# CIS565-Fall-2014/Project3-Pathtracer

Measured on NVIDIA B200. Metric: path segments per second, reference sample scene 800x800, 5000 spp, 8 bounces, higher is better.
Workload: dtype f32

## Files before the change

project3-pathtracer_b200/csrc/pt_api.cu:

```cuda
#include "../../include/pt_b200.h"
#include "pt_kernels.cuh"

#include <nvtx3/nvToolsExt.h>

#include <cmath>
#include <cstdarg>
#include <cstdio>
#include <cstring>
#include <string>
#include <algorithm>
#include <atomic>
#include <thread>
#include <functional>
#include <vector>

using namespace ptd;

struct NvtxRange {
  explicit NvtxRange(const char* name) { nvtxRangePushA(name); }
  ~NvtxRange() { nvtxRangePop(); }
};

static thread_local std::string g_err;
extern "C" void pt_set_error_(const char* fmt, ...) {
// ... 28 lines not shown
  int sm_count = 0;
  cudaStream_t own_stream = nullptr, stream = nullptr;
  cudaEvent_t ev0 = nullptr, ev1 = nullptr;
  bool timed = false;
  int n_geoms = 0, n_mats = 0;
  float4* d_rows = nullptr;
  int2* d_meta = nullptr;
  float4* d_normals = nullptr;
  float4* d_mats = nullptr;
  float4* d_lights = nullptr;
  float* d_light_k = nullptr;
  int n_lights = 0;
  bool nee = false;
  float4* d_filt = nullptr;
  int2* d_filt_ids = nullptr;
  FiltSoA filt{};
  int filt_cap = 0;
  float4* d_bvh_nodes = nullptr;
  float4* d_bvh_leaves = nullptr;
  int2* d_bvh_meta = nullptr;
  BvhSoA bvh{};
  float filter_scale = 1.0f;
  std::vector<pt_static_geom> h_geoms;
  GeomSoA g{};
  RaygenConsts cam{};
  uint32_t W = 0, H = 0, npix = 0;
  uint64_t wf_capacity = 0;
  uint32_t band_pixels = 0;
#ifndef PT_WF_SLOTS
#define PT_WF_SLOTS 2
// ... 531 lines not shown

template <bool F, bool L>
static int setup_variant(pt_context* c, int slot) {
  int per_sm = 0, per_sm_nee = 0;
  constexpr bool N = NeeOf<F, L>::value;
  if (c->mode) {
    CU(cudaFuncSetAttribute(k_bounce_bvh<L>, cudaFuncAttributeMaxDynamicSharedMemorySize, (int)kBvhSmemBytes));
    CU(cudaOccupancyMaxActiveBlocksPerMultiprocessor(&per_sm, k_bounce_bvh<L>, kBvhThreads, kBvhSmemBytes));
    CU(cudaFuncSetAttribute(k_bounce_bvh<L, N>, cudaFuncAttributeMaxDynamicSharedMemorySize, (int)kBvhSmemBytes));
    CU(cudaOccupancyMaxActiveBlocksPerMultiprocessor(&per_sm_nee, k_bounce_bvh<L, N>, kBvhThreads, kBvhSmemBytes));
  } else {
    CU(cudaFuncSetAttribute(k_bounce<F, L>, cudaFuncAttributeMaxDynamicSharedMemorySize, (int)c->smem_bytes));
    CU(cudaOccupancyMaxActiveBlocksPerMultiprocessor(&per_sm, k_bounce<F, L>, kBounceThreads, c->smem_bytes));
    CU(cudaFuncSetAttribute(k_bounce<F, L, N>, cudaFuncAttributeMaxDynamicSharedMemorySize, (int)c->smem_bytes));
    CU(cudaOccupancyMaxActiveBlocksPerMultiprocessor(&per_sm_nee, k_bounce<F, L, N>, kBounceThreads, c->smem_bytes));
  }
  if (per_sm < 1 || per_sm_nee < 1) { pt_set_error_("k_bounce does not fit on an SM"); return PT_ERR_CUDA; }
  c->grid_blocks[slot] = per_sm * c->sm_count;
  c->grid_blocks_nee[slot] = per_sm_nee * c->sm_count;
  return PT_OK;
}

template <bool L>
static int setup_variant_q(pt_context* c, int slot) {
  int per_sm = 0, per_sm_nee = 0;
  constexpr bool N = true;
  CU(cudaFuncSetAttribute(k_bounce_q<L>, cudaFuncAttributeMaxDynamicSharedMemorySize, (int)c->q_smem_total));
  CU(cudaFuncSetAttribute(k_bounce_q<L>, cudaFuncAttributePreferredSharedMemoryCarveout, cudaSharedmemCarveoutMaxShared));
  CU(cudaOccupancyMaxActiveBlocksPerMultiprocessor(&per_sm, k_bounce_q<L>, kQThreads, c->q_smem_total));
  CU(cudaFuncSetAttribute(k_bounce_q<L, N>, cudaFuncAttributeMaxDynamicSharedMemorySize, (int)c->q_smem_total));
// ... 86 lines not shown
  if (c->d_bvh_leaves) CU(cudaFree(c->d_bvh_leaves));
  if (c->d_bvh_meta) CU(cudaFree(c->d_bvh_meta));
  c->d_bvh_nodes = nullptr; c->d_bvh_leaves = nullptr; c->d_bvh_meta = nullptr;
  c->bvh = BvhSoA{};
  if (!F.leaf_meta.empty()) {
    CU(cudaMalloc(&c->d_bvh_nodes, F.nodes.size() * sizeof(float4)));
    CU(cudaMalloc(&c->d_bvh_leaves, F.leaves.size() * sizeof(float4)));
    CU(cudaMalloc(&c->d_bvh_meta, F.leaf_meta.size() * sizeof(int2)));
    CU(cudaMemcpy(c->d_bvh_nodes, F.nodes.data(), F.nodes.size() * sizeof(float4), cudaMemcpyHostToDevice));
    CU(cudaMemcpy(c->d_bvh_leaves, F.leaves.data(), F.leaves.size() * sizeof(float4), cudaMemcpyHostToDevice));
    CU(cudaMemcpy(c->d_bvh_meta, F.leaf_meta.data(), F.leaf_meta.size() * sizeof(int2), cudaMemcpyHostToDevice));
    c->bvh.nodes = c->d_bvh_nodes; c->bvh.leaves = c->d_bvh_leaves; c->bvh.leaf_meta = c->d_bvh_meta;
    c->bvh.n_leaves = (int)F.leaf_meta.size(); c->bvh.ew_c_max = F.ew_c_max; c->bvh.ew_w_max = F.ew_w_max;
    c->bvh.root = F.root;
  }
  return PT_OK;
}

static int upload_scene(pt_context* c, const pt_static_geom* geoms, int n_geoms, const pt_material* mats, int n_mats,
                        const pt_camera_data* cam, const pt_lens* lens, bool first) {
  if (!geoms || n_geoms <= 0 || !mats || n_mats <= 0 || !cam) {
    pt_set_error_("geoms, materials and camera are required and must be non-empty");
    return PT_ERR_INVALID;
  }
  const int Wi = (int)cam->resolution[0], Hi = (int)cam->resolution[1];
  if (Wi <= 0 || Hi <= 0 || (uint64_t)Wi * (uint64_t)Hi > (1ull << 31)) {
    pt_set_error_("bad resolution %d x %d", Wi, Hi);
    return PT_ERR_INVALID;
  }
  if (!first && ((uint32_t)Wi != c->W || (uint32_t)Hi != c->H)) {
// ... 71 lines not shown
    c->geom_smem = filt_smem_bytes(cap);
    c->mode = mode;
    c->smem_bytes = mode == 0 ? c->geom_smem : kBvhSmemBytes;
    int rc;
    if ((rc = setup_variant<true, false>(c, 0))) return rc;
    if ((rc = setup_variant<true, true>(c, 1))) return rc;
    if ((rc = setup_variant<false, false>(c, 2))) return rc;
    if ((rc = setup_variant<false, true>(c, 3))) return rc;
    if (mode == 0) {
      c->q_smem_total = c->geom_smem + q_smem_bytes();
      if ((rc = setup_variant_q<false>(c, 0))) return rc;
      if ((rc = setup_variant_q<true>(c, 1))) return rc;
    }
    CU(cudaFuncSetAttribute(k_intersect_list, cudaFuncAttributeMaxDynamicSharedMemorySize, (int)c->geom_smem));
  }
  return PT_OK;
}

static size_t state_bytes(uint64_t cap) { return (((size_t)cap * (7 * sizeof(float4))) + 255) & ~(size_t)255; }
static int alloc_wavefront(pt_context* c, uint64_t max_paths) {
  uint64_t spp = max_paths / c->npix;
  if (spp < 1) spp = 1;
  const uint64_t cap = spp * c->npix;
  if (cap > 0xFFFFFF00ull) { pt_set_error_("wavefront of %llu paths exceeds 2^32", (unsigned long long)cap); return PT_ERR_INVALID; }
  if (cap == c->wf_capacity) return PT_OK;
  int n_slots = pt_context::kSlots;
  if (const char* env = getenv("PT_B200_SLOTS")) n_slots = atoi(env) >= 2 ? pt_context::kSlots : 1;
  if (n_slots > 1 && !c->wf_stream[0]) {
    CU(cudaEventCreateWithFlags(&c->ev_fork, cudaEventDisableTiming));
    for (int i = 0; i < pt_context::kSlots; i++) {
      CU(cudaStreamCreateWithFlags(&c->wf_stream[i], cudaStreamNonBlocking));
// ... 21 lines not shown
  return PT_OK;
}

extern "C" int pt_context_destroy(pt_context* c) {
  if (!c) return PT_OK;
  cudaSetDevice(c->device);
  cudaStream_t streams[] = {c->stream, c->ahead_stream, c->copy_stream, c->wf_stream[0], c->wf_stream[1], c->own_stream};
  for (cudaStream_t st : streams)
    if (st) cudaStreamSynchronize(st);
  const bool dbg = getenv("PT_B200_DEBUG_DESTROY") != nullptr;
  auto chk = [&](cudaError_t e, const char* what) {
    if (e != cudaSuccess && dbg) fprintf(stderr, "pt_context_destroy: %s -> %s\n", what, cudaGetErrorString(e));
  };
#define PT_FREE(p) chk(cudaFree(p), #p)
  PT_FREE(c->d_rows); PT_FREE(c->d_meta); PT_FREE(c->d_normals); PT_FREE(c->d_mats); PT_FREE(c->d_lights); PT_FREE(c->d_state);
  PT_FREE(c->d_filt); PT_FREE(c->d_filt_ids); PT_FREE(c->d_bvh_nodes); PT_FREE(c->d_bvh_leaves); PT_FREE(c->d_bvh_meta);
  PT_FREE(c->d_ctrl); PT_FREE(c->d_live); PT_FREE(c->d_accum); PT_FREE(c->d_rgb); PT_FREE(c->d_rgba8);
  PT_FREE(c->d_scratch); PT_FREE(c->d_light_k); PT_FREE(c->d_shadow);
  PT_FREE(c->d_slab); PT_FREE(c->d_means); PT_FREE(c->d_base[0]); PT_FREE(c->d_base[1]);
#undef PT_FREE
  for (int i = 0; i < pt_context::kSlots; i++) {
    if (c->wf_stream[i]) chk(cudaStreamDestroy(c->wf_stream[i]), "wf_stream");
    if (c->ev_join[i]) chk(cudaEventDestroy(c->ev_join[i]), "ev_join");
  }
  if (c->ev_fork) chk(cudaEventDestroy(c->ev_fork), "ev_fork");
  if (c->ahead_stream) chk(cudaStreamDestroy(c->ahead_stream), "ahead_stream");
  if (c->copy_stream) chk(cudaStreamDestroy(c->copy_stream), "copy_stream");
  if (c->ev_res) chk(cudaEventDestroy(c->ev_res), "ev_res");
  if (c->ev_copy) chk(cudaEventDestroy(c->ev_copy), "ev_copy");
  for (int i = 0; i < 2; i++) {
    if (c->ev_ready[i]) chk(cudaEventDestroy(c->ev_ready[i]), "ev_ready");
// ... 119 lines not shown
    if (nee) k_bounce_q<L, N><<<gq, kQThreads, c->q_smem_total, st>>>(P);
    else k_bounce_q<L><<<gq, kQThreads, c->q_smem_total, st>>>(P);
  } else if (c->mode) {
    if (F) {
      const uint32_t blocks = (n_upper + 255u) / 256u, most = (uint32_t)c->sm_count * 8u;
      k_raygen_wf<<<blocks < most ? (blocks ? blocks : 1u) : most, 256, 0, st>>>(P);
      c->launches++;
    }
    const uint32_t ctas = (n_upper + kPoolMin * (kBvhThreads / 32) - 1) / (kPoolMin * (kBvhThreads / 32));
    if (ctas < grid) grid = ctas ? ctas : 1;
    if (nee) k_bounce_bvh<L, N><<<grid, kBvhThreads, kBvhSmemBytes, st>>>(P);
    else k_bounce_bvh<L><<<grid, kBvhThreads, kBvhSmemBytes, st>>>(P);
  } else {
    const uint32_t ctas = (n_upper + kBounceThreads - 1) / kBounceThreads;
    if (ctas < grid) grid = ctas ? ctas : 1;
    if (nee) k_bounce<F, L, N><<<grid, kBounceThreads, c->smem_bytes, st>>>(P);
    else k_bounce<F, L><<<grid, kBounceThreads, c->smem_bytes, st>>>(P);
  }
  c->launches++;
  return cudaGetLastError();
}

static int ensure_shadow(pt_context* c) {
  if (!(c->d_shadow && c->shadow_cap == c->wf_capacity && c->shadow_slots == c->n_slots)) {
    if (c->d_shadow) CU(cudaFree(c->d_shadow));
    c->d_shadow = nullptr; c->shadow_cap = 0;
    if (cudaMalloc(&c->d_shadow, (size_t)c->n_slots * 4 * c->wf_capacity * sizeof(float4)) != cudaSuccess) {
      const cudaError_t e = cudaGetLastError();
      c->d_shadow = nullptr;
      pt_set_error_("cudaMalloc of the shadow-ray queues (%llu paths) failed: %s", (unsigned long long)c->wf_capacity, cudaGetErrorString(e));
      return PT_ERR_CUDA;
    }
// ... 65 lines not shown
    const int sl = (int)(wf % (uint64_t)slots_used);
    cudaStream_t st = forked ? c->wf_stream[sl] : stream0;
    float4* S = reinterpret_cast<float4*>(reinterpret_cast<char*>(c->d_state) + (size_t)sl * state_bytes(cap));
    WfCtrl* ctrl = c->d_ctrl + sl;
    const uint32_t ns = (n_samples - s0 < spp_wf) ? (n_samples - s0) : spp_wf;
    const uint32_t n_first = ns * band;
    CU(cudaMemsetAsync(ctrl, 0, sizeof(WfCtrl), st));
    for (int depth = 0; depth < max_depth; depth++) {
      BounceParams P;
      const int in = depth & 1, outb = in ^ 1;
      P.in_o = S + (3 * in + 0) * cap; P.in_d = S + (3 * in + 1) * cap; P.in_t = S + (3 * in + 2) * cap;
      P.out_o = S + (3 * outb + 0) * cap; P.out_d = S + (3 * outb + 1) * cap; P.out_t = S + (3 * outb + 2) * cap;
      P.accum = accum; P.acc_s0 = acc_s0; P.acc_stride = acc_stride;
      P.g = c->g; P.n_geoms = c->n_geoms;
      P.normals = c->d_normals;
      P.filt = c->filt; P.filt_cap = c->filt_cap;
      P.bvh = c->bvh;
      P.bvh_res = S + 6 * cap;
      float4* const SQ = nee_on ? c->d_shadow + (size_t)sl * 4 * cap : nullptr;
      P.sq_o = SQ; P.sq_d = SQ ? SQ + cap : nullptr; P.sq_t = SQ ? SQ + 2 * cap : nullptr; P.sq_x = SQ ? SQ + 3 * cap : nullptr;
      P.mats = c->d_mats;
      P.lights = c->d_lights; P.n_lights = c->n_lights; P.light_k = c->d_light_k;
      P.cam = c->cam;
      P.ctrl = ctrl;
      P.depth = (uint32_t)depth;
      P.keys = philox_keys(seed);
      P.first_sample = first_sample + s0;
      P.n_first = n_first;
      P.pix0 = pix0; P.band = band;
      P.div_band = make_fastdiv(band);
      P.q_offset = (uint32_t)c->geom_smem;
// ... 297 lines not shown
  CU(cudaMemcpyAsync(&fb, dfb, sizeof(fb), cudaMemcpyDeviceToHost, c->stream));
  CU(cudaStreamSynchronize(c->stream));
  if (fallbacks) *fallbacks = fb;
  return PT_OK;
}
extern "C" int pt_intersect(pt_context* c, int n, const float* origin, const float* direction, int32_t* geom_id,
                            float* t, float* point, float* normal) {
  return pt_intersect_ex(c, PT_HIT_FILTERED, n, origin, direction, geom_id, t, point, normal, nullptr);
}

extern "C" int pt_set_filter_scale(pt_context* c, float scale) {
  CTX(c);
  if (!(scale >= 0.0f) || !(scale <= 1e6f)) { pt_set_error_("filter scale %g outside [0, 1e6]", (double)scale); return PT_ERR_INVALID; }
  CU(cudaStreamSynchronize(c->stream));
  c->filter_scale = scale;
  return upload_filter(c);
}

extern "C" int pt_filter_stats(pt_context* c, uint64_t* fallbacks) {
  CTX(c);
  if (!fallbacks) { pt_set_error_("fallbacks is NULL"); return PT_ERR_INVALID; }
  unsigned long long h = 0;
  CU(cudaMemcpyAsync(&h, c->d_live + kMaxDepth, sizeof(h), cudaMemcpyDeviceToHost, c->stream));
  CU(cudaStreamSynchronize(c->stream));
  *fallbacks = h;
  return PT_OK;
}

extern "C" int pt_filter_retries(pt_context* c, uint64_t* retries) {
  CTX(c);
  if (!retries) { pt_set_error_("retries is NULL"); return PT_ERR_INVALID; }
// ... 283 lines not shown
```

project3-pathtracer_b200/csrc/pt_filter.cuh:

```cuda
#pragma once
#include "pt_device.cuh"

namespace ptd {

__device__ __forceinline__ float mufu_rcp(float x) { float y; asm("rcp.approx.ftz.f32 %0, %1;" : "=f"(y) : "f"(x)); return y; }
__device__ __forceinline__ float mufu_sqrt(float x) { float y; asm("sqrt.approx.ftz.f32 %0, %1;" : "=f"(y) : "f"(x)); return y; }

constexpr int kFiltRows = 10;
constexpr int kFiltClasses = 4;
struct FiltSoA {
  const float4* rows;
  const int2* ids;
  int end[kFiltClasses];
  float r_scene;
};
__host__ __device__ inline size_t filt_smem_bytes(int cap) { return (size_t)cap * kFiltRows * sizeof(float4); }
__device__ __forceinline__ void stage_filt(const FiltSoA& g, int first, int count, float4* smem) {
  for (int i = threadIdx.x; i < count * kFiltRows; i += blockDim.x) smem[i] = g.rows[(size_t)first * kFiltRows + i];
}

typedef float2 f2;
__device__ __forceinline__ f2 bc2(float x) { return make_float2(x, x); }
__device__ __forceinline__ f2 lo2(float4 v) { return make_float2(v.x, v.y); }
__device__ __forceinline__ f2 hi2(float4 v) { return make_float2(v.z, v.w); }
// ... 39 lines not shown
  const bool first = lo < b.lo1, second = !first && lo < b.lo2;
  b.lo3 = first || second ? b.lo2 : fminf(b.lo3, lo);
  b.lo2 = first ? b.lo1 : (second ? lo : b.lo2);
  b.k2 = first ? b.k1 : (second ? k : b.k2);
  b.lo1 = first ? lo : b.lo1;
  b.k1 = first ? k : b.k1;
}
__device__ __forceinline__ void scan_take(ScanBest& b, float lo, int k) {
  lo = fmaxf(lo, 0.0f);
  const bool better = lo < b.lo1;
  b.lo2 = fminf(b.lo2, better ? b.lo1 : lo);
  b.k1 = better ? k : b.k1;
  b.lo1 = fminf(b.lo1, lo);
}

#define PT_FILT_TRANSFORM(V, R)                                                                          \
  const float4 Q0 = (V)[0], Q1 = (V)[1], Q2 = (V)[2], Q3 = (V)[3], Q4 = (V)[4], Q5 = (V)[5];             \
  const f2 rox = fma2(lo2(Q0), bc2((R).o.x), fma2(hi2(Q0), bc2((R).o.y), fma2(lo2(Q1), bc2((R).o.z), hi2(Q1)))); \
  const f2 roy = fma2(lo2(Q2), bc2((R).o.x), fma2(hi2(Q2), bc2((R).o.y), fma2(lo2(Q3), bc2((R).o.z), hi2(Q3)))); \
  const f2 roz = fma2(lo2(Q4), bc2((R).o.x), fma2(hi2(Q4), bc2((R).o.y), fma2(lo2(Q5), bc2((R).o.z), hi2(Q5)))); \
  const f2 rwx = fma2(lo2(Q0), bc2((R).d.x), fma2(hi2(Q0), bc2((R).d.y), mul2(lo2(Q1), bc2((R).d.z))));          \
  const f2 rwy = fma2(lo2(Q2), bc2((R).d.x), fma2(hi2(Q2), bc2((R).d.y), mul2(lo2(Q3), bc2((R).d.z))));          \
  const f2 rwz = fma2(lo2(Q4), bc2((R).d.x), fma2(hi2(Q4), bc2((R).d.y), mul2(lo2(Q5), bc2((R).d.z))));

#define PT_SPHERE_HALF(H)                                                                             \
  const float sd_##H = mufu_sqrt(disc.H), ia_##H = mufu_rcp(a.H);                                     \
  const bool miss_##H = (disc.H < 0.0f) || ((sd_##H - b.H) * ia_##H < 0.0f);  \
  const float lo_##H = __fmaf_rn((-b.H - sd_##H) * ia_##H, r.dl, -ew.H);
#define PT_BOX_HALF(H)                                                                                \
  const float tnear_##H = fmaxf(fmaxf(nx.H, ny.H), nz.H), tfar_##H = fminf(fminf(fx.H, fy.H), fz.H);  \
  const bool miss_##H = (tnear_##H > tfar_##H) || (tfar_##H < 0.0f);  \
  const float lo_##H = __fmaf_rn(tnear_##H, r.dl, -ew.H);
template <typename Sink>
__device__ __forceinline__ void filter_scan_to(const float4* v, int first, int last, const int end[kFiltClasses],
                                               const ScanRay& r, Sink& sink) {
  int i = first;
  const f2 w2 = bc2(r.w);
  for (const int e = min(last, end[0]); i < e; i++, v += kFiltRows) {
    const float4 C0 = v[0], C1 = v[1], C2 = v[2], C3 = v[3];
    const f2 ocx = __fadd2_rn(bc2(r.o.x), neg2(lo2(C0))), ocy = __fadd2_rn(bc2(r.o.y), neg2(hi2(C0))),
             ocz = __fadd2_rn(bc2(r.o.z), neg2(lo2(C1)));
    const f2 b = fma2(ocx, bc2(r.d.x), fma2(ocy, bc2(r.d.y), mul2(ocz, bc2(r.d.z))));
    const f2 oc2 = fma2(ocx, ocx, fma2(ocy, ocy, mul2(ocz, ocz)));
    const f2 R2 = fma2(hi2(C2), oc2, fma2(lo2(C2), w2, hi2(C1)));
    const f2 nc = __fadd2_rn(R2, neg2(oc2));
    const f2 disc = fma2(bc2(r.a), nc, mul2(b, b));
    if (disc.x < 0.0f && disc.y < 0.0f) continue;
    const f2 ew = fma2(hi2(C3), w2, lo2(C3));
    const f2 a = bc2(r.a);
    PT_SPHERE_HALF(x)
    PT_SPHERE_HALF(y)
    sink(lo_x, miss_x, lo_y, miss_y, i);
  }
  for (const int e = min(last, end[1]); i < e; i++, v += kFiltRows) {
    PT_FILT_TRANSFORM(v, r)
    const float4 K0 = v[6], K1 = v[7];
    const f2 a = fma2(rwx, rwx, fma2(rwy, rwy, mul2(rwz, rwz)));
    const f2 b = fma2(rox, rwx, fma2(roy, rwy, mul2(roz, rwz)));
    const f2 ro2 = fma2(rox, rox, fma2(roy, roy, mul2(roz, roz)));
    const f2 R2 = fma2(lo2(K1), ro2, fma2(hi2(K0), w2, lo2(K0)));
    const f2 nc = __fadd2_rn(R2, neg2(ro2));
    const f2 disc = fma2(a, nc, mul2(b, b));
    if (disc.x < 0.0f && disc.y < 0.0f) continue;
    const f2 ew = fma2(lo2(v[8]), w2, hi2(K1));
    PT_SPHERE_HALF(x)
    PT_SPHERE_HALF(y)
    sink(lo_x, miss_x, lo_y, miss_y, i);
  }
  for (const int e = min(last, end[2]); i < e; i++, v += kFiltRows) {
    const float4 C0 = v[0], C1 = v[1], C2 = v[2], C3 = v[3], C4 = v[4];
    const f2 cx = fma2(lo2(C0), bc2(r.id.x), bc2(-r.od.x)), cy = fma2(hi2(C0), bc2(r.id.y), bc2(-r.od.y)),
             cz = fma2(lo2(C1), bc2(r.id.z), bc2(-r.od.z));
    const f2 hx = fma2(lo2(C3), w2, hi2(C1)), hy = fma2(hi2(C3), w2, lo2(C2)), hz = fma2(lo2(C4), w2, hi2(C2));
    const f2 aix = bc2(fabsf(r.id.x)), aiy = bc2(fabsf(r.id.y)), aiz = bc2(fabsf(r.id.z));
    const f2 nx = fma2(hx, neg2(aix), cx), ny = fma2(hy, neg2(aiy), cy), nz = fma2(hz, neg2(aiz), cz);
    const f2 fx = fma2(hx, aix, cx), fy = fma2(hy, aiy, cy), fz = fma2(hz, aiz, cz);
    const f2 ew = fma2(lo2(v[5]), w2, hi2(C4));
    PT_BOX_HALF(x)
    PT_BOX_HALF(y)
    sink(lo_x, miss_x, lo_y, miss_y, i);
  }
  for (const int e = min(last, end[3]); i < e; i++, v += kFiltRows) {
    PT_FILT_TRANSFORM(v, r)
    const float4 K0 = v[6], K1 = v[7], K2 = v[8], K3 = v[9];
    const f2 hx = fma2(hi2(K1), w2, lo2(K0)), hy = fma2(lo2(K2), w2, hi2(K0)), hz = fma2(hi2(K2), w2, lo2(K1));
    const f2 ix = make_float2(mufu_rcp(rwx.x), mufu_rcp(rwx.y)), iy = make_float2(mufu_rcp(rwy.x), mufu_rcp(rwy.y)),
             iz = make_float2(mufu_rcp(rwz.x), mufu_rcp(rwz.y));
    const f2 cx = mul2(neg2(rox), ix), cy = mul2(neg2(roy), iy), cz = mul2(neg2(roz), iz);
    const f2 nx = fma2(hx, neg2(abs2(ix)), cx), ny = fma2(hy, neg2(abs2(iy)), cy), nz = fma2(hz, neg2(abs2(iz)), cz);
    const f2 fx = fma2(hx, abs2(ix), cx), fy = fma2(hy, abs2(iy), cy), fz = fma2(hz, abs2(iz), cz);
    const f2 ew = fma2(hi2(K3), w2, lo2(K3));
    PT_BOX_HALF(x)
    PT_BOX_HALF(y)
    sink(lo_x, miss_x, lo_y, miss_y, i);
  }
}
#undef PT_SPHERE_HALF
#undef PT_BOX_HALF
#undef PT_FILT_TRANSFORM
#ifndef PT_FILT_KEYED
#define PT_FILT_KEYED 1
#endif
struct TakeBest {
  ScanBest& b;
  __device__ __forceinline__ void operator()(float lo_a, bool miss_a, float lo_b, bool miss_b, int pair) {
    scan_take(b, miss_a ? INFINITY : lo_a, 2 * pair);
    scan_take(b, miss_b ? INFINITY : lo_b, 2 * pair + 1);
  }
};
constexpr int kKeyBits = 7;
constexpr uint32_t kKeyMask = (1u << kKeyBits) - 1u;
struct TakeBestKeyed {
  float k1 = INFINITY, k2 = INFINITY;
  static __device__ __forceinline__ float key(float lo, bool miss, uint32_t k) {
    const float v = __uint_as_float((__float_as_uint(fmaxf(lo, 0.0f)) & ~kKeyMask) | k);
    return miss ? INFINITY : v;
  }
  __device__ __forceinline__ void operator()(float lo_a, bool miss_a, float lo_b, bool miss_b, int pair) {
    const float ka = key(lo_a, miss_a, 2u * pair), kb = key(lo_b, miss_b, 2u * pair + 1u);
    const float mn = fminf(ka, kb), mx = fmaxf(ka, kb);
    k2 = fminf(fminf(k2, fmaxf(k1, mn)), mx);
    k1 = fminf(k1, mn);
  }
  __device__ __forceinline__ void finish(ScanBest& b) const {
    b.k1 = k1 < INFINITY ? (int)(__float_as_uint(k1) & kKeyMask) : -1;
    b.lo1 = __uint_as_float(__float_as_uint(k1) & ~kKeyMask);
    b.lo2 = __uint_as_float(__float_as_uint(k2) & ~kKeyMask);
  }
};
__device__ __forceinline__ void filter_scan(const float4* v, int first, int last, const int end[kFiltClasses],
                                            const ScanRay& r, ScanBest& best) {
#if PT_FILT_KEYED
  TakeBestKeyed sink;
  filter_scan_to(v, first, last, end, r, sink);
  sink.finish(best);
#else
  TakeBest sink{best};
  filter_scan_to(v, first, last, end, r, sink);
#endif
}

template <typename M>
__device__ __forceinline__ bool exact_hit(int type, float4 i0, float4 i1, float4 i2, float4 f0, float4 f1, float4 f2,
                                          f3 o, f3 d, float& dist, f3& P, int& ncode, M& m) {
  const f3 ro = mulMV(i0, i1, i2, o.x, o.y, o.z, 1.0f);
  const f3 rd = normalize(mulMV(i0, i1, i2, d.x, d.y, d.z, 0.0f), m);
  float t;
  if (type == 0) {
    const float vDot = dot(ro, rd);
    const float radicand = (float)((double)(vDot * vDot) - ((double)dot(ro, ro) - 0.25));
    if (radicand < 0) return false;
    const float sq = m.sqrt(radicand);
    const float first_term = -vDot;
// ... 71 lines not shown
```

project3-pathtracer_b200/csrc/pt_kernels.cuh:

```cuda
#pragma once
#include "pt_device.cuh"
#include "pt_filter.cuh"
#include "pt_bvh.cuh"
#include "pt_sampling.cuh"

namespace ptd {

constexpr int kMaxDepth = 64;
constexpr int kTile = 256;
#ifndef PT_BOUNCE_THREADS
#define PT_BOUNCE_THREADS 256
#endif
constexpr int kBounceThreads = PT_BOUNCE_THREADS;
#ifndef PT_MIN_BLOCKS
#define PT_MIN_BLOCKS 4
#endif

struct WfCtrl {
  uint32_t count[kMaxDepth + 1];
  uint32_t tile_ctr[kMaxDepth + 1];
  uint32_t fallbacks;
  uint32_t retries;
  unsigned long long shadow;
  uint32_t shadow_ctr[kMaxDepth + 1];
// ... 37 lines not shown
    if (pmask) break;
    look -= 32;
  }
  if (lane == 0) st_store(status + tile, st_pack(epoch, kStPrefix, exclusive + aggregate));
  return exclusive;
}

struct BounceParams {
  const float4 *in_o, *in_d, *in_t;
  float4 *out_o, *out_d, *out_t;
  float4* accum;
  GeomSoA g;
  const float4* normals;
  int n_geoms;
  FiltSoA filt;
  int filt_cap;
  BvhSoA bvh;
  float4* bvh_res;
  const float4* mats;
  const float4* lights;
  const float* light_k;
  int n_lights;
  RaygenConsts cam;
  WfCtrl* ctrl;
  uint32_t depth;
  PhiloxKeys keys;
  uint32_t first_sample, n_first;
  uint32_t pix0, band;
  FastDiv div_band;
  float4 *sq_o, *sq_d, *sq_t, *sq_x;
  uint32_t q_offset;
// ... 207 lines not shown
      if (NEE && PT_NEE_QUEUE) slot = __shfl_sync(0xffffffffu, W->pend_raw, 0) + rank;
    } else {
      slot = __shfl_sync(0xffffffffu, base_raw, 0) + rank;
      if (alive) {
        PT_CHECK(slot < P.cap);
        __stcs(io.out_o + slot, make_float4(o.x, o.y, o.z, __uint_as_float(pixel)));
        __stcs(io.out_d + slot, make_float4(d.x, d.y, d.z, __uint_as_float(sample)));
        __stcs(io.out_t + slot, make_float4(thr.x, thr.y, thr.z, sampled ? cos_s : 0.0f));
      }
    }
    if (NEE && (PT_NEE_QUEUE ? ballot != 0u : __any_sync(0xffffffffu, sampled)))
      direct_light<TABLE, LINEAR>(P, io, fs, lane, sampled, alive, slot, ns, o, thr, pixel, sample);
  }
}

template <bool FIRST, bool LAST, bool NEE>
__device__ __forceinline__ void bounce_fused(const BounceParams& P, const DepthIO& io, const float4* fs, uint32_t lane) {
  const uint32_t n_in = FIRST ? P.n_first : P.ctrl->count[io.depth];
  if (FIRST && blockIdx.x == 0 && threadIdx.x == 0) P.ctrl->count[0] = n_in;
  const uint32_t n_units = (n_in + kUnit - 1) / kUnit;
  uint32_t* const ticket = &P.ctrl->tile_ctr[io.depth];

  uint32_t next_raw = 0;
  if (lane == 0) next_raw = atom_add_u32(ticket, 1u);

  for (;;) {
    const uint32_t unit0 = __shfl_sync(0xffffffffu, next_raw, 0) * kTicketUnits;
    if (unit0 >= n_units) break;
    if (lane == 0) next_raw = atom_add_u32(ticket, 1u);
#pragma unroll 1
    for (uint32_t unit = unit0; unit < min(unit0 + kTicketUnits, n_units); unit++) {
// ... 12 lines not shown
      } else {
        const float4 a = __ldcs(io.in_o + idx), b = __ldcs(io.in_d + idx), c = __ldcs(io.in_t + idx);
        o = mk(a.x, a.y, a.z); pixel = __float_as_uint(a.w);
        d = mk(b.x, b.y, b.z); sample = __float_as_uint(b.w);
        thr = mk(c.x, c.y, c.z);
        if (NEE) cos_b = c.w;
      }
    }

    Hit h;
    h.t = INFINITY; h.id = -1; h.p = mk(0, 0, 0); h.ncode = 0;
    if (valid) {
      ScanBest best;
      scan_init(best);
      const ScanRay ray = make_scan_ray(o, d, P.filt.r_scene, P.filt.end[2] > P.filt.end[1]);
      filter_scan(fs, 0, P.filt.end[3], P.filt.end, ray, best);
      if (resolve_scan(best, P.filt, P.g, P.n_geoms, o, d, h)) atomicAdd(&P.ctrl->fallbacks, 1u);
    }

    shade_and_compact<LAST, true, NEE>(P, io, fs, lane, valid && h.id >= 0, h, o, d, thr, pixel, sample, cos_b);
    }
  }
}

template <bool FIRST, bool LAST, bool NEE = false>
__global__ void __launch_bounds__(kBounceThreads, PT_MIN_BLOCKS) k_bounce(const __grid_constant__ BounceParams P) {
  extern __shared__ __align__(16) unsigned char smem_raw[];
  stage_filt(P.filt, 0, P.filt.end[3], reinterpret_cast<float4*>(smem_raw));
  __syncthreads();
  bounce_fused<FIRST, LAST, NEE>(P, depth_io(P), reinterpret_cast<const float4*>(smem_raw), threadIdx.x & 31u);
}

constexpr int kQCap = 96;
#ifndef PT_Q_PREFETCH
#define PT_Q_PREFETCH 1
#endif
#ifndef PT_Q_PREFETCH_EARLY
#define PT_Q_PREFETCH_EARLY 1
#endif
#ifndef PT_Q_DEFER_OUT
#define PT_Q_DEFER_OUT 1
#endif
struct QWarp {
  float4 o[kQCap];
  float4 d[kQCap];
// ... 487 lines not shown
    __syncwarp();
  }
}

constexpr float kQSurvivalMax = 0.93f;
__global__ void k_accum_counts(const WfCtrl* ctrl, unsigned long long* live_total, int max_depth, volatile int* policy) {
  int d = threadIdx.x;
  if (d < max_depth) atomicAdd(live_total + d, (unsigned long long)ctrl->count[d]);
  if (d == 0) atomicAdd(live_total + kMaxDepth, (unsigned long long)ctrl->fallbacks);
  if (d == 1) atomicAdd(live_total + kMaxDepth + 1, ctrl->shadow);
  if (d == 2) atomicAdd(live_total + kMaxDepth + 2, (unsigned long long)ctrl->retries);
  if (policy && d >= 1 && d < max_depth && ctrl->count[d - 1] >= 4096u)
    policy[d] = (float)ctrl->count[d] < kQSurvivalMax * (float)ctrl->count[d - 1] ? 1 : 2;
}

__global__ void k_normal_table(GeomSoA g, int n_geoms, const float4* mats, float4* tab) {
  const int i = blockIdx.x * blockDim.x + threadIdx.x;
  if (i >= n_geoms) return;
  const float4 f0 = g.fwd0[i], f1 = g.fwd1[i], f2 = g.fwd2[i];
  Hit h;
  h.t = 0.0f; h.id = i; h.p = mk(0, 0, 0);
  for (int face = 0; face < 6; face++) {
    h.ncode = (face % 3) | (face >= 3 ? 4 : 0);
    const f3 n = hit_normal(f0, f1, f2, h);
    tab[(size_t)i * kNormalRows + face] = make_float4(n.x, n.y, n.z, 0.0f);
    f3 p1, p2;
    float4* fr = tab + (size_t)i * kNormalRows + kFrameRow0 + 4 * face;
    hemisphere_frame(n, p1, p2);
    fr[0] = make_float4(p1.x, p1.y, p1.z, 0.0f); fr[1] = make_float4(p2.x, p2.y, p2.z, 0.0f);
    hemisphere_frame(neg(n), p1, p2);
// ... 350 lines not shown
```

Before: 29000.

## Precompute eye-origin filter rows for primary rays in pinhole scenes

When the camera is a pinhole (aperture zero) and no BVH is used, the code precomputes per-pair filter rows specialised to the fixed eye origin. An EYE-templated first-bounce kernel then reads these origin-dependent terms (transformed origin, |oc|^2 terms, half extents, ew) instead of recomputing them per ray. This cuts arithmetic in the primary-ray filter scan only, at the cost of extra kernel instantiations, an extra device buffer, and recomputing the rows whenever the scene or filter scale changes. A standalone microbenchmark file is also added.

```diff
diff --git a/profiles/microbench/const_rows.cu b/profiles/microbench/const_rows.cu
--- /dev/null
+++ b/profiles/microbench/const_rows.cu
@@ -0,0 +1,32 @@
+#include <cuda_runtime.h>
+struct Rows { float4 r[19 * 10]; int n; };
+__device__ __forceinline__ float2 lo2(float4 v) { return make_float2(v.x, v.y); }
+__device__ __forceinline__ float2 hi2(float4 v) { return make_float2(v.z, v.w); }
+__global__ void k_fixed(const __grid_constant__ Rows R, const float4* in, float2* out) {
+  const float4 a = in[threadIdx.x + blockIdx.x * blockDim.x];
+  const float2 x = make_float2(a.x, a.y), y = make_float2(a.z, a.w);
+  float2 t = __ffma2_rn(x, lo2(R.r[3]), y);
+  t = __ffma2_rn(t, y, hi2(R.r[3]));
+  t = __ffma2_rn(t, make_float2(R.r[4].x, R.r[4].x), x);
+  t = __fadd2_rn(t, lo2(R.r[4]));
+  out[threadIdx.x] = __fmul2_rn(t, hi2(R.r[4]));
+}
+__global__ void k_loop(const __grid_constant__ Rows R, const float4* in, float* out) {
+  const float4 a = in[threadIdx.x + blockIdx.x * blockDim.x];
+  const float2 o = make_float2(a.x, a.x), d = make_float2(a.y, a.y);
+  float2 acc = make_float2(0.f, 0.f);
+#pragma unroll 1
+  for (int i = 0; i < R.n; i++) {
+    const float4 C0 = R.r[i * 10], C1 = R.r[i * 10 + 1];
+    float2 t = __ffma2_rn(lo2(C0), o, hi2(C0));
+    t = __ffma2_rn(lo2(C1), t, hi2(C1));
+    if (t.x < 0.f && t.y < 0.f) continue;
+    acc = __ffma2_rn(t, d, acc);
+  }
+  out[threadIdx.x] = acc.x + acc.y;
+}
+__global__ void k_block(const __grid_constant__ Rows R, const float4* in, float2* out) {
+  const float4 a = in[threadIdx.x + blockIdx.x * blockDim.x];
+  const float4 C = R.r[blockIdx.x];
+  out[threadIdx.x] = __ffma2_rn(make_float2(a.x, a.y), lo2(C), hi2(C));
+}
diff --git a/project3-pathtracer_b200/csrc/pt_api.cu b/project3-pathtracer_b200/csrc/pt_api.cu
--- a/project3-pathtracer_b200/csrc/pt_api.cu
+++ b/project3-pathtracer_b200/csrc/pt_api.cu
@@ -66,6 +66,8 @@
   bool nee = false;
   float4* d_filt = nullptr;
   int2* d_filt_ids = nullptr;
+  float4* d_filt_eye = nullptr;
+  bool eye_rows = false;
   FiltSoA filt{};
   int filt_cap = 0;
   float4* d_bvh_nodes = nullptr;
@@ -627,6 +629,13 @@
     CU(cudaOccupancyMaxActiveBlocksPerMultiprocessor(&per_sm, k_bounce<F, L>, kBounceThreads, c->smem_bytes));
     CU(cudaFuncSetAttribute(k_bounce<F, L, N>, cudaFuncAttributeMaxDynamicSharedMemorySize, (int)c->smem_bytes));
     CU(cudaOccupancyMaxActiveBlocksPerMultiprocessor(&per_sm_nee, k_bounce<F, L, N>, kBounceThreads, c->smem_bytes));
+    int per_sm_eye = 0, per_sm_nee_eye = 0;
+    CU(cudaFuncSetAttribute(k_bounce<F, L, false, F>, cudaFuncAttributeMaxDynamicSharedMemorySize, (int)c->smem_bytes));
+    CU(cudaOccupancyMaxActiveBlocksPerMultiprocessor(&per_sm_eye, k_bounce<F, L, false, F>, kBounceThreads, c->smem_bytes));
+    CU(cudaFuncSetAttribute(k_bounce<F, L, N, F>, cudaFuncAttributeMaxDynamicSharedMemorySize, (int)c->smem_bytes));
+    CU(cudaOccupancyMaxActiveBlocksPerMultiprocessor(&per_sm_nee_eye, k_bounce<F, L, N, F>, kBounceThreads, c->smem_bytes));
+    if (per_sm_eye < per_sm) per_sm = per_sm_eye;
+    if (per_sm_nee_eye < per_sm_nee) per_sm_nee = per_sm_nee_eye;
   }
   if (per_sm < 1 || per_sm_nee < 1) { pt_set_error_("k_bounce does not fit on an SM"); return PT_ERR_CUDA; }
   c->grid_blocks[slot] = per_sm * c->sm_count;
@@ -743,6 +752,20 @@
     c->bvh.n_leaves = (int)F.leaf_meta.size(); c->bvh.ew_c_max = F.ew_c_max; c->bvh.ew_w_max = F.ew_w_max;
     c->bvh.root = F.root;
   }
+  return PT_OK;
+}
+
+static int upload_eye_rows(pt_context* c) {
+  c->eye_rows = false;
+  const int n_pairs = c->filt.end[3];
+  if (c->bvh.n_leaves > 0 || !(c->cam.aperture == 0.0f) || n_pairs < 1) return PT_OK;
+  if (c->d_filt_eye) CU(cudaFree(c->d_filt_eye));
+  c->d_filt_eye = nullptr;
+  CU(cudaMalloc(&c->d_filt_eye, (size_t)n_pairs * kFiltRows * sizeof(float4)));
+  k_eye_rows<<<(n_pairs + 127) / 128, 128, 0, c->stream>>>(c->filt, c->cam.eye, c->d_filt_eye);
+  CU(cudaGetLastError());
+  CU(cudaStreamSynchronize(c->stream));
+  c->eye_rows = true;
   return PT_OK;
 }
 
@@ -844,7 +867,7 @@
     }
     CU(cudaFuncSetAttribute(k_intersect_list, cudaFuncAttributeMaxDynamicSharedMemorySize, (int)c->geom_smem));
   }
-  return PT_OK;
+  return upload_eye_rows(c);
 }
 
 static size_t state_bytes(uint64_t cap) { return (((size_t)cap * (7 * sizeof(float4))) + 255) & ~(size_t)255; }
@@ -896,7 +919,7 @@
   };
 #define PT_FREE(p) chk(cudaFree(p), #p)
   PT_FREE(c->d_rows); PT_FREE(c->d_meta); PT_FREE(c->d_normals); PT_FREE(c->d_mats); PT_FREE(c->d_lights); PT_FREE(c->d_state);
-  PT_FREE(c->d_filt); PT_FREE(c->d_filt_ids); PT_FREE(c->d_bvh_nodes); PT_FREE(c->d_bvh_leaves); PT_FREE(c->d_bvh_meta);
+  PT_FREE(c->d_filt); PT_FREE(c->d_filt_ids); PT_FREE(c->d_filt_eye); PT_FREE(c->d_bvh_nodes); PT_FREE(c->d_bvh_leaves); PT_FREE(c->d_bvh_meta);
   PT_FREE(c->d_ctrl); PT_FREE(c->d_live); PT_FREE(c->d_accum); PT_FREE(c->d_rgb); PT_FREE(c->d_rgba8);
   PT_FREE(c->d_scratch); PT_FREE(c->d_light_k); PT_FREE(c->d_shadow);
   PT_FREE(c->d_slab); PT_FREE(c->d_means); PT_FREE(c->d_base[0]); PT_FREE(c->d_base[1]);
@@ -1046,8 +1069,16 @@
   } else {
     const uint32_t ctas = (n_upper + kBounceThreads - 1) / kBounceThreads;
     if (ctas < grid) grid = ctas ? ctas : 1;
-    if (nee) k_bounce<F, L, N><<<grid, kBounceThreads, c->smem_bytes, st>>>(P);
-    else k_bounce<F, L><<<grid, kBounceThreads, c->smem_bytes, st>>>(P);
+    if (F && c->eye_rows && (PT_NEE_QUEUE || !nee)) {
+      BounceParams Pe = P;
+      Pe.filt.rows = c->d_filt_eye;
+      if (nee) k_bounce<F, L, N, F><<<grid, kBounceThreads, c->smem_bytes, st>>>(Pe);
+      else k_bounce<F, L, false, F><<<grid, kBounceThreads, c->smem_bytes, st>>>(Pe);
+    } else if (nee) {
+      k_bounce<F, L, N><<<grid, kBounceThreads, c->smem_bytes, st>>>(P);
+    } else {
+      k_bounce<F, L><<<grid, kBounceThreads, c->smem_bytes, st>>>(P);
+    }
   }
   c->launches++;
   return cudaGetLastError();
@@ -1143,7 +1174,7 @@
       P.accum = accum; P.acc_s0 = acc_s0; P.acc_stride = acc_stride;
       P.g = c->g; P.n_geoms = c->n_geoms;
       P.normals = c->d_normals;
-      P.filt = c->filt; P.filt_cap = c->filt_cap;
+      P.filt = c->filt;
       P.bvh = c->bvh;
       P.bvh_res = S + 6 * cap;
       float4* const SQ = nee_on ? c->d_shadow + (size_t)sl * 4 * cap : nullptr;
@@ -1471,7 +1502,8 @@
   if (!(scale >= 0.0f) || !(scale <= 1e6f)) { pt_set_error_("filter scale %g outside [0, 1e6]", (double)scale); return PT_ERR_INVALID; }
   CU(cudaStreamSynchronize(c->stream));
   c->filter_scale = scale;
-  return upload_filter(c);
+  if (int rc = upload_filter(c)) return rc;
+  return upload_eye_rows(c);
 }
 
 extern "C" int pt_filter_stats(pt_context* c, uint64_t* fallbacks) {
diff --git a/project3-pathtracer_b200/csrc/pt_filter.cuh b/project3-pathtracer_b200/csrc/pt_filter.cuh
--- a/project3-pathtracer_b200/csrc/pt_filter.cuh
+++ b/project3-pathtracer_b200/csrc/pt_filter.cuh
@@ -77,14 +77,77 @@
   b.lo1 = fminf(b.lo1, lo);
 }
 
-#define PT_FILT_TRANSFORM(V, R)                                                                          \
-  const float4 Q0 = (V)[0], Q1 = (V)[1], Q2 = (V)[2], Q3 = (V)[3], Q4 = (V)[4], Q5 = (V)[5];             \
-  const f2 rox = fma2(lo2(Q0), bc2((R).o.x), fma2(hi2(Q0), bc2((R).o.y), fma2(lo2(Q1), bc2((R).o.z), hi2(Q1)))); \
-  const f2 roy = fma2(lo2(Q2), bc2((R).o.x), fma2(hi2(Q2), bc2((R).o.y), fma2(lo2(Q3), bc2((R).o.z), hi2(Q3)))); \
-  const f2 roz = fma2(lo2(Q4), bc2((R).o.x), fma2(hi2(Q4), bc2((R).o.y), fma2(lo2(Q5), bc2((R).o.z), hi2(Q5)))); \
-  const f2 rwx = fma2(lo2(Q0), bc2((R).d.x), fma2(hi2(Q0), bc2((R).d.y), mul2(lo2(Q1), bc2((R).d.z))));          \
-  const f2 rwy = fma2(lo2(Q2), bc2((R).d.x), fma2(hi2(Q2), bc2((R).d.y), mul2(lo2(Q3), bc2((R).d.z))));          \
-  const f2 rwz = fma2(lo2(Q4), bc2((R).d.x), fma2(hi2(Q4), bc2((R).d.y), mul2(lo2(Q5), bc2((R).d.z))));
+__device__ __forceinline__ void filt_ro(const float4* v, f3 o, f2& rox, f2& roy, f2& roz) {
+  const float4 Q0 = v[0], Q1 = v[1], Q2 = v[2], Q3 = v[3], Q4 = v[4], Q5 = v[5];
+  rox = fma2(lo2(Q0), bc2(o.x), fma2(hi2(Q0), bc2(o.y), fma2(lo2(Q1), bc2(o.z), hi2(Q1))));
+  roy = fma2(lo2(Q2), bc2(o.x), fma2(hi2(Q2), bc2(o.y), fma2(lo2(Q3), bc2(o.z), hi2(Q3))));
+  roz = fma2(lo2(Q4), bc2(o.x), fma2(hi2(Q4), bc2(o.y), fma2(lo2(Q5), bc2(o.z), hi2(Q5))));
+}
+__device__ __forceinline__ void filt_rw(const float4* v, f3 d, f2& rwx, f2& rwy, f2& rwz) {
+  const float4 Q0 = v[0], Q1 = v[1], Q2 = v[2], Q3 = v[3], Q4 = v[4], Q5 = v[5];
+  rwx = fma2(lo2(Q0), bc2(d.x), fma2(hi2(Q0), bc2(d.y), mul2(lo2(Q1), bc2(d.z))));
+  rwy = fma2(lo2(Q2), bc2(d.x), fma2(hi2(Q2), bc2(d.y), mul2(lo2(Q3), bc2(d.z))));
+  rwz = fma2(lo2(Q4), bc2(d.x), fma2(hi2(Q4), bc2(d.y), mul2(lo2(Q5), bc2(d.z))));
+}
+__device__ __forceinline__ void filt_origin0(const float4* v, f3 o, f2 w2, f2& ocx, f2& ocy, f2& ocz, f2& nc) {
+  const float4 C0 = v[0], C1 = v[1], C2 = v[2];
+  ocx = __fadd2_rn(bc2(o.x), neg2(lo2(C0))); ocy = __fadd2_rn(bc2(o.y), neg2(hi2(C0)));
+  ocz = __fadd2_rn(bc2(o.z), neg2(lo2(C1)));
+  const f2 oc2 = fma2(ocx, ocx, fma2(ocy, ocy, mul2(ocz, ocz)));
+  const f2 R2 = fma2(hi2(C2), oc2, fma2(lo2(C2), w2, hi2(C1)));
+  nc = __fadd2_rn(R2, neg2(oc2));
+}
+__device__ __forceinline__ f2 filt_nc1(const float4* v, f2 w2, f2 rox, f2 roy, f2 roz) {
+  const float4 K0 = v[6], K1 = v[7];
+  const f2 ro2 = fma2(rox, rox, fma2(roy, roy, mul2(roz, roz)));
+  const f2 R2 = fma2(lo2(K1), ro2, fma2(hi2(K0), w2, lo2(K0)));
+  return __fadd2_rn(R2, neg2(ro2));
+}
+__device__ __forceinline__ void filt_half2(const float4* v, f2 w2, f2& hx, f2& hy, f2& hz) {
+  const float4 C1 = v[1], C2 = v[2], C3 = v[3], C4 = v[4];
+  hx = fma2(lo2(C3), w2, hi2(C1)); hy = fma2(hi2(C3), w2, lo2(C2)); hz = fma2(lo2(C4), w2, hi2(C2));
+}
+__device__ __forceinline__ void filt_half3(const float4* v, f2 w2, f2& hx, f2& hy, f2& hz) {
+  const float4 K0 = v[6], K1 = v[7], K2 = v[8];
+  hx = fma2(hi2(K1), w2, lo2(K0)); hy = fma2(lo2(K2), w2, hi2(K0)); hz = fma2(hi2(K2), w2, lo2(K1));
+}
+template <int K>
+__device__ __forceinline__ f2 filt_ew(const float4* v, f2 w2) {
+  if (K == 0) return fma2(hi2(v[3]), w2, lo2(v[3]));
+  if (K == 1) return fma2(lo2(v[8]), w2, hi2(v[7]));
+  if (K == 2) return fma2(lo2(v[5]), w2, hi2(v[4]));
+  return fma2(hi2(v[9]), w2, lo2(v[9]));
+}
+
+__device__ __forceinline__ void eye_rows_of_pair(const FiltSoA& f, int i, f3 eye, float4* e) {
+  const float4* const v = f.rows + (size_t)i * kFiltRows;
+  for (int k = 0; k < kFiltRows; k++) e[k] = v[k];
+  const ScanRay r = make_scan_ray(eye, mk(0, 0, 1), f.r_scene, false);
+  const f2 w2 = bc2(r.w);
+  const f2 z = bc2(0.0f);
+  f2 ax, ay, az, nc, ew;
+  if (i < f.end[0]) {
+    filt_origin0(v, r.o, w2, ax, ay, az, nc);
+    ew = filt_ew<0>(v, w2);
+    e[0] = make_float4(ax.x, ax.y, ay.x, ay.y); e[1] = make_float4(az.x, az.y, nc.x, nc.y); e[2] = make_float4(ew.x, ew.y, z.x, z.y);
+  } else if (i < f.end[1]) {
+    filt_ro(v, r.o, ax, ay, az);
+    nc = filt_nc1(v, w2, ax, ay, az);
+    ew = filt_ew<1>(v, w2);
+    e[6] = make_float4(ax.x, ax.y, ay.x, ay.y); e[7] = make_float4(az.x, az.y, nc.x, nc.y); e[8] = make_float4(ew.x, ew.y, z.x, z.y);
+  } else if (i < f.end[2]) {
+    filt_half2(v, w2, ax, ay, az);
+    ew = filt_ew<2>(v, w2);
+    e[1].z = ax.x; e[1].w = ax.y; e[2] = make_float4(ay.x, ay.y, az.x, az.y); e[3] = make_float4(ew.x, ew.y, z.x, z.y);
+  } else {
+    f2 hx, hy, hz;
+    filt_ro(v, r.o, ax, ay, az);
+    filt_half3(v, w2, hx, hy, hz);
+    ew = filt_ew<3>(v, w2);
+    e[6] = make_float4(ax.x, ax.y, ay.x, ay.y); e[7] = make_float4(az.x, az.y, hx.x, hx.y); e[8] = make_float4(hy.x, hy.y, hz.x, hz.y);
+    e[9] = make_float4(ew.x, ew.y, z.x, z.y);
+  }
+}
 
 #define PT_SPHERE_HALF(H)                                                                             \
   const float sd_##H = mufu_sqrt(disc.H), ia_##H = mufu_rcp(a.H);                                     \
@@ -94,65 +157,87 @@
   const float tnear_##H = fmaxf(fmaxf(nx.H, ny.H), nz.H), tfar_##H = fminf(fminf(fx.H, fy.H), fz.H);  \
   const bool miss_##H = (tnear_##H > tfar_##H) || (tfar_##H < 0.0f);  \
   const float lo_##H = __fmaf_rn(tnear_##H, r.dl, -ew.H);
-template <typename Sink>
+template <bool EYE, typename Sink>
 __device__ __forceinline__ void filter_scan_to(const float4* v, int first, int last, const int end[kFiltClasses],
                                                const ScanRay& r, Sink& sink) {
   int i = first;
   const f2 w2 = bc2(r.w);
   for (const int e = min(last, end[0]); i < e; i++, v += kFiltRows) {
-    const float4 C0 = v[0], C1 = v[1], C2 = v[2], C3 = v[3];
-    const f2 ocx = __fadd2_rn(bc2(r.o.x), neg2(lo2(C0))), ocy = __fadd2_rn(bc2(r.o.y), neg2(hi2(C0))),
-             ocz = __fadd2_rn(bc2(r.o.z), neg2(lo2(C1)));
+    f2 ocx, ocy, ocz, nc;
+    if (EYE) {
+      const float4 E0 = v[0], E1 = v[1];
+      ocx = lo2(E0); ocy = hi2(E0); ocz = lo2(E1); nc = hi2(E1);
+    } else {
+      filt_origin0(v, r.o, w2, ocx, ocy, ocz, nc);
+    }
     const f2 b = fma2(ocx, bc2(r.d.x), fma2(ocy, bc2(r.d.y), mul2(ocz, bc2(r.d.z))));
-    const f2 oc2 = fma2(ocx, ocx, fma2(ocy, ocy, mul2(ocz, ocz)));
-    const f2 R2 = fma2(hi2(C2), oc2, fma2(lo2(C2), w2, hi2(C1)));
-    const f2 nc = __fadd2_rn(R2, neg2(oc2));
     const f2 disc = fma2(bc2(r.a), nc, mul2(b, b));
     if (disc.x < 0.0f && disc.y < 0.0f) continue;
-    const f2 ew = fma2(hi2(C3), w2, lo2(C3));
+    const f2 ew = EYE ? lo2(v[2]) : filt_ew<0>(v, w2);
     const f2 a = bc2(r.a);
     PT_SPHERE_HALF(x)
     PT_SPHERE_HALF(y)
     sink(lo_x, miss_x, lo_y, miss_y, i);
   }
   for (const int e = min(last, end[1]); i < e; i++, v += kFiltRows) {
-    PT_FILT_TRANSFORM(v, r)
-    const float4 K0 = v[6], K1 = v[7];
+    f2 rox, roy, roz, rwx, rwy, rwz;
+    if (EYE) {
+      const float4 E6 = v[6];
+      rox = lo2(E6); roy = hi2(E6); roz = lo2(v[7]);
+    } else {
+      filt_ro(v, r.o, rox, roy, roz);
+    }
+    filt_rw(v, r.d, rwx, rwy, rwz);
+    const f2 nc = EYE ? hi2(v[7]) : filt_nc1(v, w2, rox, roy, roz);
     const f2 a = fma2(rwx, rwx, fma2(rwy, rwy, mul2(rwz, rwz)));
     const f2 b = fma2(rox, rwx, fma2(roy, rwy, mul2(roz, rwz)));
-    const f2 ro2 = fma2(rox, rox, fma2(roy, roy, mul2(roz, roz)));
-    const f2 R2 = fma2(lo2(K1), ro2, fma2(hi2(K0), w2, lo2(K0)));
-    const f2 nc = __fadd2_rn(R2, neg2(ro2));
     const f2 disc = fma2(a, nc, mul2(b, b));
     if (disc.x < 0.0f && disc.y < 0.0f) continue;
-    const f2 ew = fma2(lo2(v[8]), w2, hi2(K1));
+    const f2 ew = EYE ? lo2(v[8]) : filt_ew<1>(v, w2);
     PT_SPHERE_HALF(x)
     PT_SPHERE_HALF(y)
     sink(lo_x, miss_x, lo_y, miss_y, i);
   }
   for (const int e = min(last, end[2]); i < e; i++, v += kFiltRows) {
-    const float4 C0 = v[0], C1 = v[1], C2 = v[2], C3 = v[3], C4 = v[4];
+    const float4 C0 = v[0], C1 = v[1];
     const f2 cx = fma2(lo2(C0), bc2(r.id.x), bc2(-r.od.x)), cy = fma2(hi2(C0), bc2(r.id.y), bc2(-r.od.y)),
              cz = fma2(lo2(C1), bc2(r.id.z), bc2(-r.od.z));
-    const f2 hx = fma2(lo2(C3), w2, hi2(C1)), hy = fma2(hi2(C3), w2, lo2(C2)), hz = fma2(lo2(C4), w2, hi2(C2));
+    f2 hx, hy, hz;
+    if (EYE) {
+      const float4 E2 = v[2];
+      hx = hi2(C1); hy = lo2(E2); hz = hi2(E2);
+    } else {
+      filt_half2(v, w2, hx, hy, hz);
+    }
     const f2 aix = bc2(fabsf(r.id.x)), aiy = bc2(fabsf(r.id.y)), aiz = bc2(fabsf(r.id.z));
     const f2 nx = fma2(hx, neg2(aix), cx), ny = fma2(hy, neg2(aiy), cy), nz = fma2(hz, neg2(aiz), cz);
     const f2 fx = fma2(hx, aix, cx), fy = fma2(hy, aiy, cy), fz = fma2(hz, aiz, cz);
-    const f2 ew = fma2(lo2(v[5]), w2, hi2(C4));
+    const f2 ew = EYE ? lo2(v[3]) : filt_ew<2>(v, w2);
     PT_BOX_HALF(x)
     PT_BOX_HALF(y)
     sink(lo_x, miss_x, lo_y, miss_y, i);
   }
   for (const int e = min(last, end[3]); i < e; i++, v += kFiltRows) {
-    PT_FILT_TRANSFORM(v, r)
-    const float4 K0 = v[6], K1 = v[7], K2 = v[8], K3 = v[9];
-    const f2 hx = fma2(hi2(K1), w2, lo2(K0)), hy = fma2(lo2(K2), w2, hi2(K0)), hz = fma2(hi2(K2), w2, lo2(K1));
+    f2 rox, roy, roz, rwx, rwy, rwz, hx, hy, hz;
+    if (EYE) {
+      const float4 E6 = v[6];
+      rox = lo2(E6); roy = hi2(E6); roz = lo2(v[7]);
+    } else {
+      filt_ro(v, r.o, rox, roy, roz);
+    }
+    filt_rw(v, r.d, rwx, rwy, rwz);
+    if (EYE) {
+      const float4 E7 = v[7], E8 = v[8];
+      hx = hi2(E7); hy = lo2(E8); hz = hi2(E8);
+    } else {
+      filt_half3(v, w2, hx, hy, hz);
+    }
     const f2 ix = make_float2(mufu_rcp(rwx.x), mufu_rcp(rwx.y)), iy = make_float2(mufu_rcp(rwy.x), mufu_rcp(rwy.y)),
              iz = make_float2(mufu_rcp(rwz.x), mufu_rcp(rwz.y));
     const f2 cx = mul2(neg2(rox), ix), cy = mul2(neg2(roy), iy), cz = mul2(neg2(roz), iz);
     const f2 nx = fma2(hx, neg2(abs2(ix)), cx), ny = fma2(hy, neg2(abs2(iy)), cy), nz = fma2(hz, neg2(abs2(iz)), cz);
     const f2 fx = fma2(hx, abs2(ix), cx), fy = fma2(hy, abs2(iy), cy), fz = fma2(hz, abs2(iz), cz);
-    const f2 ew = fma2(hi2(K3), w2, lo2(K3));
+    const f2 ew = EYE ? lo2(v[9]) : filt_ew<3>(v, w2);
     PT_BOX_HALF(x)
     PT_BOX_HALF(y)
     sink(lo_x, miss_x, lo_y, miss_y, i);
@@ -160,7 +245,6 @@
 }
 #undef PT_SPHERE_HALF
 #undef PT_BOX_HALF
-#undef PT_FILT_TRANSFORM
 #ifndef PT_FILT_KEYED
 #define PT_FILT_KEYED 1
 #endif
@@ -191,15 +275,16 @@
     b.lo2 = __uint_as_float(__float_as_uint(k2) & ~kKeyMask);
   }
 };
+template <bool EYE = false>
 __device__ __forceinline__ void filter_scan(const float4* v, int first, int last, const int end[kFiltClasses],
                                             const ScanRay& r, ScanBest& best) {
 #if PT_FILT_KEYED
   TakeBestKeyed sink;
-  filter_scan_to(v, first, last, end, r, sink);
+  filter_scan_to<EYE>(v, first, last, end, r, sink);
   sink.finish(best);
 #else
   TakeBest sink{best};
-  filter_scan_to(v, first, last, end, r, sink);
+  filter_scan_to<EYE>(v, first, last, end, r, sink);
 #endif
 }
 
diff --git a/project3-pathtracer_b200/csrc/pt_kernels.cuh b/project3-pathtracer_b200/csrc/pt_kernels.cuh
--- a/project3-pathtracer_b200/csrc/pt_kernels.cuh
+++ b/project3-pathtracer_b200/csrc/pt_kernels.cuh
@@ -75,7 +75,6 @@
   const float4* normals;
   int n_geoms;
   FiltSoA filt;
-  int filt_cap;
   BvhSoA bvh;
   float4* bvh_res;
   const float4* mats;
@@ -313,7 +312,7 @@
   }
 }
 
-template <bool FIRST, bool LAST, bool NEE>
+template <bool FIRST, bool LAST, bool NEE, bool EYE>
 __device__ __forceinline__ void bounce_fused(const BounceParams& P, const DepthIO& io, const float4* fs, uint32_t lane) {
   const uint32_t n_in = FIRST ? P.n_first : P.ctrl->count[io.depth];
   if (FIRST && blockIdx.x == 0 && threadIdx.x == 0) P.ctrl->count[0] = n_in;
@@ -356,7 +355,7 @@
       ScanBest best;
       scan_init(best);
       const ScanRay ray = make_scan_ray(o, d, P.filt.r_scene, P.filt.end[2] > P.filt.end[1]);
-      filter_scan(fs, 0, P.filt.end[3], P.filt.end, ray, best);
+      filter_scan<EYE>(fs, 0, P.filt.end[3], P.filt.end, ray, best);
       if (resolve_scan(best, P.filt, P.g, P.n_geoms, o, d, h)) atomicAdd(&P.ctrl->fallbacks, 1u);
     }
 
@@ -365,12 +364,13 @@
   }
 }
 
-template <bool FIRST, bool LAST, bool NEE = false>
+template <bool FIRST, bool LAST, bool NEE = false, bool EYE = false>
 __global__ void __launch_bounds__(kBounceThreads, PT_MIN_BLOCKS) k_bounce(const __grid_constant__ BounceParams P) {
+  static_assert(FIRST || !EYE, "eye rows serve primary rays only");
   extern __shared__ __align__(16) unsigned char smem_raw[];
   stage_filt(P.filt, 0, P.filt.end[3], reinterpret_cast<float4*>(smem_raw));
   __syncthreads();
-  bounce_fused<FIRST, LAST, NEE>(P, depth_io(P), reinterpret_cast<const float4*>(smem_raw), threadIdx.x & 31u);
+  bounce_fused<FIRST, LAST, NEE, EYE>(P, depth_io(P), reinterpret_cast<const float4*>(smem_raw), threadIdx.x & 31u);
 }
 
 constexpr int kQCap = 96;
@@ -888,6 +888,11 @@
     policy[d] = (float)ctrl->count[d] < kQSurvivalMax * (float)ctrl->count[d - 1] ? 1 : 2;
 }
 
+__global__ void k_eye_rows(FiltSoA f, f3 eye, float4* out) {
+  const int i = blockIdx.x * blockDim.x + threadIdx.x;
+  if (i < f.end[3]) eye_rows_of_pair(f, i, eye, out + (size_t)i * kFiltRows);
+}
+
 __global__ void k_normal_table(GeomSoA g, int n_geoms, const float4* mats, float4* tab) {
   const int i = blockIdx.x * blockDim.x + threadIdx.x;
   if (i >= n_geoms) return;
```

Result: faster. 29400 (median of 6 runs) (+1.4%).
